# maotian123/loc_lib

Measured on AMD Instinct MI355X. Metric: scans/sec (64x1800-pt scan vs 10M-pt map) + ICP iter ms, higher is better.
Workload: dtype f64; 1 GPU; BASELINE configs[2]: 256 scans/GPU x 115200 pts (64x1800, cityblock-v1) vs one 10000000-pt map, P2PLANE ICP, reference defaults (alpha=0.1 KD-tree ANN, eps=1e-2, max 20 iters), scans sharded by rank, no collective; includes scan H2D: every step aligns a batch copied host->HBM for it (pinned double buffer, copy stream, overlapped with the previous step); 3 alignment(s) in flight; scans_per_gpu=256, map_points=10000000, pipeline_depth=3, search_mode=tree_faithful_ann, tree_depth=30, tree_bytes=239999992

## Files before the change

include/locgpu.h:

```cpp
#ifndef LOCGPU_H_
#define LOCGPU_H_

#include <stddef.h>
#include <stdint.h>

#ifdef __cplusplus
extern "C" {
#endif

#define LOCGPU_API __attribute__((visibility("default")))

typedef struct locgpu_ctx locgpu_ctx;
typedef struct locgpu_batch locgpu_batch;

typedef enum locgpu_status {
    LOCGPU_OK = 0,
    LOCGPU_ERR_INVALID = -1,
    LOCGPU_ERR_NO_DEVICE = -2,
    LOCGPU_ERR_NO_TARGET = -3,
    LOCGPU_ERR_K_TOO_LARGE = -4,
    LOCGPU_ERR_DEPTH = -5,
    LOCGPU_ERR_OOM = -6
} locgpu_status;

// ... 185 lines not shown
LOCGPU_API int locgpu_ndt_align(locgpu_ctx* ctx, const void* src, size_t n, size_t stride_bytes, const double init_pose[7],
                                double out_pose[7], locgpu_align_stats* stats);
LOCGPU_API int locgpu_ndt_hb(locgpu_ctx* ctx, const void* src, size_t n, size_t stride_bytes, const double pose[7], double H[36], double B[6],
                             int64_t* effective_num, int* ok);
LOCGPU_API int locgpu_ndt_hb_batch(locgpu_ctx* ctx, locgpu_batch* b, const double* poses, double* hb);

LOCGPU_API int locgpu_ndt_fitness(locgpu_ctx* ctx, const void* src, size_t n, size_t stride_bytes, const double* poses, int n_poses,
                                  locgpu_fitness* out);
LOCGPU_API int locgpu_ndt_fitness_batch(locgpu_ctx* ctx, locgpu_batch* batch, const double* poses, locgpu_fitness* out);
LOCGPU_API int locgpu_ndt_fitness_resident(locgpu_ctx* ctx, const double pose[7], locgpu_fitness* out);
LOCGPU_API int locgpu_ndt_init_search(locgpu_ctx* ctx, const void* src, size_t n, size_t stride_bytes, const double* candidates, int m,
                                      const locgpu_init_search_opts* sopts, double* out_poses, locgpu_fitness* out_fit,
                                      locgpu_align_stats* stats, int* best);

LOCGPU_API int locgpu_graph_enable(locgpu_ctx* ctx, int on);

LOCGPU_API int locgpu_profile_enable(locgpu_ctx* ctx, int on);
LOCGPU_API int locgpu_profile_read(locgpu_ctx* ctx, double out[6], int reset);
LOCGPU_API int locgpu_visit_count_enable(locgpu_ctx* ctx, int on);
LOCGPU_API int locgpu_visit_count_read(locgpu_ctx* ctx, uint64_t out[4], int reset);

LOCGPU_API int locgpu_search_stats_read(locgpu_ctx* ctx, uint64_t out[4], int reset);
LOCGPU_API int locgpu_debug_batch_nn(locgpu_ctx* ctx, locgpu_batch* batch, int k, int32_t* out);

typedef struct locgpu_cloud locgpu_cloud;
typedef struct locgpu_submap locgpu_submap;
#define LOCGPU_NO_INTENSITY ((size_t)-1)

LOCGPU_API int locgpu_cloud_create(locgpu_ctx* ctx, locgpu_cloud** out);
LOCGPU_API void locgpu_cloud_destroy(locgpu_cloud* c);
LOCGPU_API int locgpu_cloud_upload(locgpu_cloud* c, const void* pts, size_t n, size_t stride_bytes, size_t intensity_offset, int is_dense);
LOCGPU_API int locgpu_cloud_info(const locgpu_cloud* c, size_t* n, int* is_dense);
LOCGPU_API int locgpu_cloud_download(const locgpu_cloud* c, void* out, size_t capacity, size_t stride_bytes, size_t intensity_offset);
LOCGPU_API int locgpu_cloud_copy(const locgpu_cloud* in, locgpu_cloud* out);

LOCGPU_API int locgpu_cloud_remove_nan(const locgpu_cloud* in, locgpu_cloud* out);
LOCGPU_API int locgpu_cloud_voxel_filter(const locgpu_cloud* in, float leaf, locgpu_cloud* out, int* passthrough);
LOCGPU_API int locgpu_cloud_crop_box(const locgpu_cloud* in, const float min_xyz[3], const float max_xyz[3], locgpu_cloud* out);
LOCGPU_API int locgpu_cloud_transform(const locgpu_cloud* in, const double pose[7], locgpu_cloud* out);
LOCGPU_API int locgpu_cloud_append(locgpu_cloud* dst, const locgpu_cloud* src);

LOCGPU_API int locgpu_icp_set_target_cloud(locgpu_ctx* ctx, const locgpu_cloud* target);
LOCGPU_API int locgpu_icp_set_target_cloud_async(locgpu_ctx* ctx, const locgpu_cloud* target);
LOCGPU_API int locgpu_ndt_set_target_cloud(locgpu_ctx* ctx, const locgpu_cloud* target, const locgpu_ndt_opts* opts);
LOCGPU_API int locgpu_icp_align_cloud(locgpu_ctx* ctx, const locgpu_cloud* src, const double init_pose[7], const locgpu_icp_opts* opts,
                                      double out_pose[7], locgpu_align_stats* stats);
// ... 62 lines not shown
```

loc_lib_amd/api.py:

```python
import ctypes
import os
import subprocess

import numpy as np

_HERE = os.path.dirname(os.path.abspath(__file__))
LIB_PATH = os.environ.get("LOCGPU_LIB") or os.path.join(_HERE, "liblocgpu.so")
CSRC = os.path.join(_HERE, "csrc")

P2P, P2LINE, P2PLANE = 0, 1, 2
P2PLANE_MAP = 5
SEARCH_TREE_FAITHFUL, SEARCH_GRID_EXACT = 0, 1
CENTER, NEARBY6 = 0, 1
DIRECT_NDT, INCREMENTAL_NDT = 1, 2

ABI_SYMBOLS = [
    "locgpu_icp_opts_default", "locgpu_ndt_opts_default", "locgpu_create", "locgpu_destroy", "locgpu_last_error",
    "locgpu_device_count", "locgpu_icp_set_target", "locgpu_icp_set_target_async", "locgpu_icp_target_info", "locgpu_knn", "locgpu_icp_hb", "locgpu_icp_align",
    "locgpu_transform_cloud", "locgpu_batch_create", "locgpu_batch_destroy", "locgpu_icp_align_batch", "locgpu_ndt_align_batch",
    "locgpu_icp_hb_batch", "locgpu_gn_update", "locgpu_ndt_set_target", "locgpu_ndt_target_info", "locgpu_ndt_dump",
    "locgpu_ndt_align", "locgpu_profile_enable", "locgpu_profile_read", "locgpu_visit_count_enable", "locgpu_visit_count_read",
    "locgpu_search_stats_read", "locgpu_debug_batch_nn", "locgpu_graph_enable",
    "locgpu_cloud_create", "locgpu_cloud_destroy", "locgpu_cloud_upload", "locgpu_cloud_info", "locgpu_cloud_download", "locgpu_cloud_copy",
    "locgpu_cloud_remove_nan", "locgpu_cloud_voxel_filter", "locgpu_cloud_crop_box", "locgpu_cloud_transform", "locgpu_cloud_append",
    "locgpu_icp_set_target_cloud", "locgpu_icp_set_target_cloud_async", "locgpu_ndt_set_target_cloud", "locgpu_icp_align_cloud", "locgpu_ndt_align_cloud",
    "locgpu_voxel_filter", "locgpu_crop_box", "locgpu_remove_nan",
    "locgpu_submap_create", "locgpu_submap_destroy", "locgpu_submap_add_keyframe", "locgpu_submap_cloud", "locgpu_submap_last_keyframe",
    "locgpu_submap_info", "locgpu_cloud_loam_extract", "locgpu_loam_extract",
    "locgpu_batch_create_empty", "locgpu_batch_upload_async", "locgpu_batch_upload_wait",
    "locgpu_bfnn_set_target", "locgpu_bfnn_knn",
    "locgpu_icp_align_batch_begin", "locgpu_ndt_align_batch_begin", "locgpu_align_batch_end",
    "locgpu_comm_unique_id", "locgpu_comm_init", "locgpu_comm_info", "locgpu_batch_create_sharded", "locgpu_icp_set_target_bcast",
    "locgpu_pool_opts_default", "locgpu_pool_create", "locgpu_pool_destroy", "locgpu_pool_submit", "locgpu_pool_wait", "locgpu_pool_info",
    "locgpu_pool_profile_read", "locgpu_pool_step", "locgpu_pool_done",
    "locgpu_icp_scan_match", "locgpu_ndt_scan_match",
    "locgpu_icp_fitness", "locgpu_icp_fitness_batch", "locgpu_icp_fitness_resident", "locgpu_batch_create_shared",
    "locgpu_init_search_opts_default", "locgpu_icp_init_search", "locgpu_pose_grid",
    "locgpu_ndt_fitness", "locgpu_ndt_fitness_batch", "locgpu_ndt_fitness_resident", "locgpu_ndt_init_search", "locgpu_ndt_hb", "locgpu_ndt_hb_batch",
    "locgpu_icp_build_map_planes", "locgpu_icp_map_planes_info", "locgpu_icp_map_planes_dump",
    "locgpu_loam_opts_default", "locgpu_loam_create", "locgpu_loam_destroy", "locgpu_loam_last_error", "locgpu_loam_set_target",
    "locgpu_loam_hb", "locgpu_loam_scan_match", "locgpu_loam_align_batch",
    "locgpu_loam_set_target_cloud", "locgpu_loam_set_target_cloud_async", "locgpu_loam_scan_match_cloud", "locgpu_loam_fitness_resident",
    "locgpu_loam_submap_create", "locgpu_loam_submap_destroy", "locgpu_loam_submap_add_keyframe", "locgpu_loam_submap_clouds", "locgpu_loam_submap_info",
    "locgpu_loam_create_on", "locgpu_loam_fitness", "locgpu_loam_fitness_cloud", "locgpu_loam_init_search", "locgpu_loam_init_search_cloud",
    "locgpu_batch_preprocess", "locgpu_batch_upload_clouds", "locgpu_batch_download_scan",
# ... 62 lines not shown
        if not os.path.exists(LIB_PATH):
            raise LocGpuError(-2, "liblocgpu.so is not built (run `python -c 'import __graft_entry__ as g; g.build()'`); no CPU fallback exists")
        L = ctypes.CDLL(LIB_PATH)
        vp, sz, i32, dbl, f32 = ctypes.c_void_p, ctypes.c_size_t, ctypes.c_int, ctypes.c_double, ctypes.c_float
        sig = {
            "locgpu_icp_opts_default": (None, [vp]), "locgpu_ndt_opts_default": (None, [vp]),
            "locgpu_create": (i32, [i32, vp]), "locgpu_destroy": (None, [vp]), "locgpu_last_error": (ctypes.c_char_p, [vp]),
            "locgpu_device_count": (i32, []),
            "locgpu_icp_set_target": (i32, [vp, vp, sz, sz]), "locgpu_icp_set_target_async": (i32, [vp, vp, sz, sz]), "locgpu_icp_target_info": (i32, [vp, vp]),
            "locgpu_knn": (i32, [vp, vp, sz, i32, i32, f32, i32, vp, vp]),
            "locgpu_icp_hb": (i32, [vp, vp, sz, sz, vp, vp, vp, vp, vp, vp]),
            "locgpu_icp_align": (i32, [vp, vp, sz, sz, vp, vp, vp, vp]),
            "locgpu_transform_cloud": (i32, [vp, vp, vp, sz, sz, vp, sz]),
            "locgpu_batch_create": (i32, [vp, vp, vp, sz, i32, vp]), "locgpu_batch_destroy": (None, [vp]),
            "locgpu_icp_align_batch": (i32, [vp, vp, vp, vp, vp, vp]), "locgpu_ndt_align_batch": (i32, [vp, vp, vp, vp, vp]),
            "locgpu_icp_align_batch_begin": (i32, [vp, vp, vp, vp]), "locgpu_ndt_align_batch_begin": (i32, [vp, vp, vp]),
            "locgpu_align_batch_end": (i32, [vp, vp, vp, vp]),
            "locgpu_icp_hb_batch": (i32, [vp, vp, vp, vp, vp]),
            "locgpu_gn_update": (i32, [vp, i32, i32, dbl, vp, vp, vp, vp]),
            "locgpu_ndt_set_target": (i32, [vp, vp, sz, sz, vp]), "locgpu_ndt_target_info": (i32, [vp, vp]),
            "locgpu_ndt_dump": (i32, [vp, vp, vp, vp, sz, vp]), "locgpu_ndt_align": (i32, [vp, vp, sz, sz, vp, vp, vp]),
            "locgpu_profile_enable": (i32, [vp, i32]), "locgpu_profile_read": (i32, [vp, vp, i32]),
            "locgpu_visit_count_enable": (i32, [vp, i32]), "locgpu_visit_count_read": (i32, [vp, vp, i32]),
            "locgpu_search_stats_read": (i32, [vp, vp, i32]), "locgpu_debug_batch_nn": (i32, [vp, vp, i32, vp]), "locgpu_graph_enable": (i32, [vp, i32]),
            "locgpu_cloud_create": (i32, [vp, vp]), "locgpu_cloud_destroy": (None, [vp]),
            "locgpu_cloud_upload": (i32, [vp, vp, sz, sz, sz, i32]), "locgpu_cloud_info": (i32, [vp, vp, vp]),
            "locgpu_cloud_download": (i32, [vp, vp, sz, sz, sz]), "locgpu_cloud_copy": (i32, [vp, vp]),
            "locgpu_cloud_remove_nan": (i32, [vp, vp]), "locgpu_cloud_voxel_filter": (i32, [vp, f32, vp, vp]),
            "locgpu_cloud_crop_box": (i32, [vp, vp, vp, vp]), "locgpu_cloud_transform": (i32, [vp, vp, vp]),
            "locgpu_cloud_append": (i32, [vp, vp]),
            "locgpu_icp_set_target_cloud": (i32, [vp, vp]), "locgpu_icp_set_target_cloud_async": (i32, [vp, vp]), "locgpu_ndt_set_target_cloud": (i32, [vp, vp, vp]),
            "locgpu_icp_align_cloud": (i32, [vp, vp, vp, vp, vp, vp]), "locgpu_ndt_align_cloud": (i32, [vp, vp, vp, vp, vp]),
            "locgpu_voxel_filter": (i32, [vp, vp, sz, sz, sz, i32, f32, vp, vp, vp]),
            "locgpu_crop_box": (i32, [vp, vp, sz, sz, sz, i32, vp, vp, vp, vp, vp]),
            "locgpu_remove_nan": (i32, [vp, vp, sz, sz, sz, i32, vp, vp, vp]),
            "locgpu_submap_create": (i32, [vp, i32, f32, vp]), "locgpu_submap_destroy": (None, [vp]),
            "locgpu_submap_add_keyframe": (i32, [vp, vp, vp]), "locgpu_submap_cloud": (i32, [vp, vp]),
            "locgpu_submap_last_keyframe": (i32, [vp, vp]), "locgpu_submap_info": (i32, [vp, vp, vp]),
            "locgpu_cloud_loam_extract": (i32, [vp, vp, i32, vp, vp]),
            "locgpu_loam_extract": (i32, [vp, vp, sz, sz, sz, i32, sz, i32, vp, vp, vp, vp, sz, sz]),
            "locgpu_batch_create_empty": (i32, [vp, i32, sz, vp]), "locgpu_batch_upload_async": (i32, [vp, vp, vp, sz]),
            "locgpu_batch_upload_wait": (i32, [vp]),
            "locgpu_comm_unique_id": (i32, [vp]), "locgpu_comm_init": (i32, [vp, i32, i32, vp]), "locgpu_comm_info": (i32, [vp, vp, vp]),
            "locgpu_batch_create_sharded": (i32, [vp, vp, vp, sz, i32, i32, i32, vp]),
            "locgpu_icp_set_target_bcast": (i32, [vp, vp, sz, sz, i32]),
            "locgpu_bfnn_set_target": (i32, [vp, vp, sz, sz]), "locgpu_bfnn_knn": (i32, [vp, vp, sz, i32, vp]),
            "locgpu_pool_opts_default": (None, [vp]), "locgpu_pool_create": (i32, [vp, vp, vp]), "locgpu_pool_destroy": (None, [vp]),
# ... 703 lines not shown

    @staticmethod
    def _marshal(scans):
        if isinstance(scans, MarshalledScans):
            return scans.scans, scans.ptrs, scans.cnts, scans.stride
        scans = [_cloud(s) for s in scans]
        if not scans:
            raise ValueError("empty batch")
        stride = next((s.strides[0] for s in scans if s.shape[0]), 16)
        if any(s.shape[0] and s.strides[0] != stride for s in scans):
            raise ValueError("all scans of a batch must share one point stride")
        ptrs = (ctypes.c_void_p * len(scans))(*[s.ctypes.data for s in scans])
        cnts = (ctypes.c_size_t * len(scans))(*[s.shape[0] for s in scans])
        return scans, ptrs, cnts, stride

    def upload_async(self, scans):
        self.upload_wait()
        scans, ptrs, cnts, stride = self._marshal(scans)
        if len(scans) != self.n_local:
            raise ValueError("upload_async needs %d scans" % self.n_local)
        self._keep = (scans, ptrs, cnts)
        self.ctx._check(lib().locgpu_batch_upload_async(self._h, ptrs, cnts, stride))

    def upload_wait(self):
        if self._keep is not None:
            rc = lib().locgpu_batch_upload_wait(self._h)
            self._keep = None
            self.ctx._check(rc)

    def preprocess(self, leaf, out=None):
        self.upload_wait()
        dst = self if out is None else out
        dst.upload_wait()
        counts, status = np.zeros(self.n_local, np.int32), np.zeros(self.n_local, np.int32)
        rc = lib().locgpu_batch_preprocess(self._h, float(leaf), dst._h, counts.ctypes.data, status.ctypes.data)
        if rc != 0:
            err = LocGpuError(rc, lib().locgpu_last_error(self.ctx._h).decode())
            err.counts = counts
            raise err
        return counts, status

    def loam_extract(self, rings, num_scan, edge, surf):
        self.upload_wait()
        edge.upload_wait()
        surf.upload_wait()
        rings = [np.ascontiguousarray(r, dtype=np.uint8) if r is not None else None for r in rings]
# ... 283 lines not shown
```

loc_lib_amd/csrc/context.hpp:

```cpp
#pragma once
#include <hip/hip_runtime.h>

#include <string>
#include <vector>

#include "../../include/locgpu.h"
#include "batch_upload.hpp"
#include "device_buffer.hpp"
#include "device_math.hpp"
#include "grid_kernels.hpp"
#include "icp_kernels.hpp"

#include "host_worker.hpp"

struct NdtTable;
namespace locgpu {
struct IncNdtState;
struct FilterScratch;
struct LoamScratch;
struct BatchFilterScratch;
struct BatchLoamScratch;
struct MergeScratch;
}

// ... 5 lines not shown
    bool grid = false;
    bool ndt() const { return method_is_ndt(prm.method); }
    int k() const { return method_k(prm.method); }
    bool operator==(const AlignSpec& o) const { return prm == o.prm && alpha == o.alpha && grid == o.grid; }
};
constexpr int kNdtOptDirect = 1, kNdtOptIncremental = 2;
constexpr int kNearbyCenter = 0, kNearby6 = 1;
constexpr int ndt_n_nearby(int nearby_type) { return nearby_type == kNearbyCenter ? 1 : 7; }
struct StageEvents {
    std::vector<Event> ev;
    size_t used = 0;
    int mode = 0;
    void mark(hipStream_t s, bool search_edge = false);
    void collect(locgpu_ctx* ctx, bool ndt);
};
}

struct locgpu_ctx {
    int device = 0;
    hipStream_t stream = nullptr;
    static constexpr int kSlots = 3;
    hipStream_t slot_stream[kSlots] = {};
    int next_slot = 0;
    hipStream_t copy_stream = nullptr;
    locgpu::Event foreign_ev;
    hipStream_t comm_stream = nullptr;
    locgpu::Uploader* up = nullptr;
    locgpu::PendingTarget* target_scratch = nullptr;
    locgpu::PendingTarget* pending_target = nullptr;
    std::string err;

    locgpu::DevBuf<uint2> d_tree;
    size_t tree_slots = 0, num_leaves = 0, num_nodes = 0, num_points = 0;
    int depth = 0;
    bool tree_bounded = true;
    unsigned long long target_epoch = 0;

    locgpu::DevBuf<uint32_t> d_leaf_slots;

    locgpu::DevBuf<double> d_planes;
    size_t planes_rows = 0;
    bool planes_ready = false;
    long long planes_valid = 0;
    locgpu::DevBuf<unsigned long long> d_planes_count;
    locgpu_batch* planes_ws = nullptr;

// ... 16 lines not shown
    locgpu_batch* single = nullptr;
    size_t single_cap = 0;
    locgpu_batch* search = nullptr;
    locgpu::HostWorker* worker = nullptr;

    void* comm = nullptr;
    int comm_rank = 0, comm_world = 1;

    int profile = 0;
    double prof_ms[3] = {0, 0, 0};
    long long prof_n[3] = {0, 0, 0};
    bool use_graph = false;
    bool count_visits = false;
    locgpu::DevBuf<unsigned long long> d_visits;
    locgpu::DevBuf<uint32_t> d_touched;
    size_t touched_words = 0;
    locgpu::DevBuf<unsigned long long> d_search_stats;
};

struct locgpu_batch {
    locgpu_ctx* ctx = nullptr;
    int slot = 0;
    hipStream_t stream = nullptr;
    int n_scans = 0, max_n = 0, blocks_per_scan = 0;
    int n_total = 0, first = 0;
    bool sharded = false;
    locgpu::DevBuf<double> d_acc;
    size_t pitch = 0;
    locgpu::DevBuf<float4> d_src;
    locgpu::DevBuf<int> d_counts;
    locgpu::DevBuf<locgpu::PoseState> d_state;
    locgpu::DevBuf<uint32_t> d_nn;
    bool shared_src = false;
    locgpu::DevBuf<int> d_src_of;
    int cap_scans = 0, split_scans = 0;
    size_t cap_points = 0;
    const float4* d_src_ext = nullptr;
    bool counters_clean = false;
    int last_iterations = -1;
    locgpu::DevBuf<double> d_partials;
    locgpu::DevBuf<double> d_hb;
    locgpu::DevBuf<uint32_t> d_redo_list;
    locgpu::DevBuf<unsigned int> d_redo_count;
    locgpu::DevBuf<uint32_t> d_redo_list2;
    locgpu::DevBuf<uint32_t> d_grid_qkey;
    locgpu::DevBuf<uint2> d_grid_sorted;
// ... 59 lines not shown
```

loc_lib_amd/csrc/gn_driver.hip:

```cpp
#include <algorithm>
#include <chrono>
#include <cmath>
#include <cstdlib>
#include <cstring>
#include <string>
#include <thread>

#include "batch_upload.hpp"
#include "env.hpp"
#include "gn_driver.hpp"
#include "ndt_inc.hpp"
#include "ndt_kernels.hpp"

namespace locgpu {

namespace {
inline int next_chunk(const locgpu_batch* b) { return b->n_total == 1 ? 2 : kNextChunk; }
inline int first_chunk_len(const locgpu_batch* b) {
    if (b->n_total != 1 || b->sharded || b->last_iterations < 0) return kFirstChunk;
    return std::min(kLongFirstChunk, std::max(3, b->last_iterations + 1));
}

}

SearchArgs make_search_args(const locgpu_ctx* ctx, const locgpu_batch* b, const float4* src, const PoseState* st, int k, float alpha_eff, bool skip_nonfinite) {
    SearchArgs sa{ctx->d_tree, ctx->tree_slots * sizeof(uint64_t), ctx->depth, src, b->d_counts, st, b->d_nn, b->pitch, b->max_n, b->n_scans, k, alpha_eff,
                  skip_nonfinite ? 1 : 0, nullptr, b->d_redo_list, b->d_redo_count, b->d_redo_list2, b->d_redo_count + 1, ctx->d_search_stats};
    if (!ctx->tree_bounded) sa.redo_list = nullptr;
    return sa;
}

void init_state(PoseState& ps, const double pose[7]) {
    std::memset(&ps, 0, sizeof(ps));
    for (int i = 0; i < 4; ++i) ps.q[i] = pose[i];
    for (int i = 0; i < 3; ++i) ps.t[i] = pose[4 + i];
// ... 189 lines not shown
}

static int ensure_graphs(locgpu_ctx* ctx, locgpu_batch* b, const AlignSpec& spec) {
    const void* target = !spec.ndt() ? (const void*)ctx->d_tree : (spec.prm.method == kMethodNdtInc ? inc_ndt_table_ptr(ctx->inc) : (const void*)ctx->ndt->d_rec);
    if (b->graph_exec && b->graph_spec == spec && b->graph_target == target && b->graph_epoch == ctx->target_epoch) return LOCGPU_OK;
    const int first = std::min(kFirstChunk, spec.prm.max_iteration);
    if (b->graph_exec) { (void)hipGraphExecDestroy(b->graph_exec); b->graph_exec = nullptr; }
    if (b->graph_exec_next) { (void)hipGraphExecDestroy(b->graph_exec_next); b->graph_exec_next = nullptr; }
    int rc = capture_chunk(ctx, b, spec, first, true, &b->graph_exec);
    if (rc == LOCGPU_OK && spec.prm.max_iteration > first) rc = capture_chunk(ctx, b, spec, next_chunk(b), false, &b->graph_exec_next);
    if (rc != LOCGPU_OK) return rc;
    b->graph_spec = spec; b->graph_target = target;
    b->graph_epoch = ctx->target_epoch;
    return LOCGPU_OK;
}

static int enqueue_chunk(locgpu_ctx* ctx, locgpu_batch* b, bool first_chunk) {
    locgpu_batch::Pending& P = b->pending;
    const GnParams& prm = P.spec.prm;
    hipStream_t s = b->stream;
    if (P.graph) {
        LOCGPU_HIP(ctx, hipGraphLaunch(first_chunk ? b->graph_exec : b->graph_exec_next, s));
        P.launched += first_chunk ? std::min(kFirstChunk, prm.max_iteration) : next_chunk(b);
        return LOCGPU_OK;
    }
    if (first_chunk) LOCGPU_HIP(ctx, hipMemcpyAsync(b->d_state, b->h_state, b->n_total * sizeof(PoseState), hipMemcpyHostToDevice, s));
    IterLauncher it{ctx, b, P.spec};
    if (!first_chunk && !P.spec.ndt() && b->n_scans > 1) {
        int na = 0;
        for (int i = 0; i < b->n_scans; ++i)
            if (!b->h_state[b->first + i].done) b->h_active[na++] = i;
        if (na > 0 && na < b->n_scans) {
            LOCGPU_HIP(ctx, hipMemcpyAsync(b->d_active, b->h_active, (size_t)na * sizeof(int), hipMemcpyHostToDevice, s));
            it.active = b->d_active;
            it.n_active = na;
        }
    }
    const int todo = std::min(first_chunk ? first_chunk_len(b) : next_chunk(b), prm.max_iteration - P.launched);
    for (int c = 0; c < todo; ++c)
        if (!it.launch(1)) return LOCGPU_ERR_NO_DEVICE;
    P.launched += todo;
    if (it.replicated_on_comm_stream) {
        LOCGPU_HIP(ctx, hipEventRecord(b->ev_reduced, ctx->comm_stream));
        LOCGPU_HIP(ctx, hipStreamWaitEvent(s, b->ev_reduced, 0));
    }
    LOCGPU_HIP(ctx, hipMemcpyAsync(b->h_state, b->d_state, b->n_total * sizeof(PoseState), hipMemcpyDeviceToHost, s));
    return LOCGPU_OK;
}

inline int pace_ahead() {
    static const int v = std::max(0, std::min(8, env_int("LOCGPU_PACE_AHEAD", 1)));
    return v;
}

static int paced_launch(locgpu_ctx* ctx, locgpu_batch* b, int upto) {
    locgpu_batch::Pending& P = b->pending;
    IterLauncher it{ctx, b, P.spec};
    const GnPost post{reinterpret_cast<GnPostRecord*>(b->h_post.get()), b->h_post + locgpu_batch::kPostWord, b->post_call};
    it.post = &post;
    while (P.launched < upto) {
        if (!it.launch(1)) return LOCGPU_ERR_NO_DEVICE;
        P.launched++;
    }
    return LOCGPU_OK;
}

constexpr int kPacedTimeoutS = 30;
static int paced_wait(locgpu_ctx* ctx, locgpu_batch* b, int seen, unsigned long long* out) {
    auto fresh = [&](unsigned long long* w_out) {
// ... 16 lines not shown
        return true;
    };
    const auto t0 = std::chrono::steady_clock::now();
    for (unsigned long spins = 1;; ++spins) {
        if (fresh(out)) return LOCGPU_OK;
#if defined(__x86_64__)
        __builtin_ia32_pause();
#endif
        if ((spins & 0xffff) == 0 && std::chrono::steady_clock::now() - t0 > std::chrono::milliseconds(200)) {
            const hipError_t q = hipStreamQuery(b->stream);
            if (q == hipErrorNotReady) {
                if (std::chrono::steady_clock::now() - t0 > std::chrono::seconds(kPacedTimeoutS))
                    return fail(ctx, LOCGPU_ERR_NO_DEVICE, "paced alignment: no post from the solve kernel within the time-out (the stream is still busy)");
                std::this_thread::yield();
                continue;
            }
            if (q != hipSuccess) { hip_ok(ctx, q, "paced alignment"); return LOCGPU_ERR_NO_DEVICE; }
            if (fresh(out)) return LOCGPU_OK;
            return fail(ctx, LOCGPU_ERR_NO_DEVICE, "paced alignment: the stream is idle and the solve kernel's post has not arrived");
        }
    }
}

int align_begin(locgpu_ctx* ctx, locgpu_batch* b, const double* init_poses, const AlignSpec& spec, bool blocking) {
    const GnParams& prm = spec.prm;
    const bool ndt = spec.ndt();
    LOCGPU_HIP(ctx, hipSetDevice(ctx->device));
    locgpu_batch::Pending& P = b->pending;
    if (P.active) return fail(ctx, LOCGPU_ERR_INVALID, "align: an alignment of this batch has been begun and not finished");
    if (!ndt) { const int grc = ensure_grid_lists(ctx, b, spec); if (grc != LOCGPU_OK) return grc; }
    { const int urc = batch_ready(ctx, b); if (urc != LOCGPU_OK) return urc; }
    P.spec = spec;
    P.graph = ctx->use_graph && !ctx->count_visits && !b->sharded && prm.max_iteration > 0;
    P.launched = 0;
    b->stage_ev.used = 0;
    P.init_poses.assign(init_poses, init_poses + 7 * (size_t)b->n_total);
    init_states(b, init_poses);
    if (!ndt && !b->counters_clean) LOCGPU_HIP(ctx, hipMemsetAsync(b->d_redo_count, 0, 4 * sizeof(unsigned int), b->stream));
    b->counters_clean = false;
    if (P.graph) { const int rc = ensure_graphs(ctx, b, spec); if (rc != LOCGPU_OK) return rc; }
    P.paced = blocking && !P.graph && b->n_total == 1 && !b->sharded && !ctx->profile && !ctx->count_visits && prm.max_iteration > 0 && pace_ahead() > 0 && !spec.grid;
    if (P.paced) {
        if (!b->h_post) {
            LOCGPU_HIP(ctx, b->h_post.alloc(256 / sizeof(unsigned long long), hipHostMallocCoherent));
            std::memset(b->h_post, 0, 256);
        }
        b->post_call++;
        LOCGPU_HIP(ctx, hipMemcpyAsync(b->d_state, b->h_state, sizeof(PoseState), hipMemcpyHostToDevice, b->stream));
        const int rc = paced_launch(ctx, b, std::min(prm.max_iteration, 1 + pace_ahead()));
        if (rc != LOCGPU_OK) { (void)hipStreamSynchronize(b->stream); return rc; }
    } else if (prm.max_iteration > 0) {
        const int rc = enqueue_chunk(ctx, b, true);
        if (rc != LOCGPU_OK) return rc;
    }
    P.active = true;
    return LOCGPU_OK;
}

int align_finish(locgpu_ctx* ctx, locgpu_batch* b, double* out_poses, locgpu_align_stats* stats) {
    LOCGPU_HIP(ctx, hipSetDevice(ctx->device));
    locgpu_batch::Pending& P = b->pending;
    if (!P.active) return fail(ctx, LOCGPU_ERR_INVALID, "align: no alignment of this batch has been begun");
    const int max_iteration = P.spec.prm.max_iteration;
    P.active = false;
    if (P.paced) {
        int seen = 0;
        for (;;) {
            unsigned long long w = 0;
            int rc = paced_wait(ctx, b, seen, &w);
            if (rc == LOCGPU_OK) {
                seen = (int)((w & 0xffffffffull) >> 1);
                if ((w & 1ull) || seen >= max_iteration) break;
                rc = paced_launch(ctx, b, std::min(max_iteration, seen + 1 + pace_ahead()));
            }
            if (rc != LOCGPU_OK) { (void)hipStreamSynchronize(b->stream); return rc; }
        }
        b->paced_tail = true;
    }
    while (!P.paced && max_iteration > 0) {
        LOCGPU_HIP(ctx, hipStreamSynchronize(b->stream));
        b->stage_ev.collect(ctx, P.spec.ndt());
        bool all_done = true;
        for (int i = 0; i < b->n_total; ++i)
            if (!b->h_state[i].done) { all_done = false; break; }
        if (all_done || P.launched >= max_iteration) break;
        const int rc = enqueue_chunk(ctx, b, false);
        if (rc != LOCGPU_OK) {
            (void)hipStreamSynchronize(b->stream);
            return rc;
        }
    }
    for (int i = 0; i < b->n_total; ++i) write_scan_result(b->h_state[i], P.init_poses.data() + 7 * (size_t)i, out_poses + 7 * (size_t)i, stats ? stats + i : nullptr);
    b->counters_clean = !P.spec.ndt() && !ctx->count_visits && !P.spec.grid && !b->sharded;
    if (b->n_total == 1 && max_iteration > 0) b->last_iterations = b->h_state[0].iterations;
    return LOCGPU_OK;
}

int run_align(locgpu_ctx* ctx, locgpu_batch* b, const double* init_poses, const AlignSpec& spec, double* out_poses, locgpu_align_stats* stats) {
    const int rc = align_begin(ctx, b, init_poses, spec,  true);
    return rc != LOCGPU_OK ? rc : align_finish(ctx, b, out_poses, stats);
}

constexpr size_t kPlaneChunk = (size_t)1 << 20;
int ensure_map_planes(locgpu_ctx* ctx) {
    if (ctx->planes_ready) return LOCGPU_OK;
    LOCGPU_HIP(ctx, hipSetDevice(ctx->device));
    hipStream_t s = ctx->stream;
    const size_t rows = ctx->tree_slots / 2 + 2;
    if (rows * 4 > ctx->d_planes.cap() && !hip_ok(ctx, ctx->d_planes.alloc(with_headroom(rows) * 4), "hipMalloc map planes")) return LOCGPU_ERR_OOM;
    if (!hip_ok(ctx, ctx->d_planes_count.reserve(1), "hipMalloc map planes")) return LOCGPU_ERR_OOM;
    LOCGPU_HIP(ctx, hipMemsetAsync(ctx->d_planes, 0xFF, rows * 4 * sizeof(double), s));
    LOCGPU_HIP(ctx, hipMemsetAsync(ctx->d_planes_count, 0, sizeof(unsigned long long), s));
    unsigned long long n_valid = 0;
    if (ctx->num_leaves >= 5) {
        const size_t chunk = std::min(ctx->num_leaves, kPlaneChunk);
        locgpu_batch* w = ctx->planes_ws;
        if (!w || (size_t)w->max_n < chunk) {
            if (w) { free_batch(w); ctx->planes_ws = nullptr; }
            const int next_slot = ctx->next_slot;
            const int rc = alloc_batch(ctx, 1, chunk, &ctx->planes_ws);
            ctx->next_slot = next_slot;
            if (rc != LOCGPU_OK) return rc;
            w = ctx->planes_ws;
            w->slot = 0;
            w->stream = s;
        }
        const double identity[7] = {0, 0, 0, 1, 0, 0, 0};
        init_states(w, identity);
        LOCGPU_HIP(ctx, hipMemsetAsync(w->d_redo_count, 0, 4 * sizeof(unsigned int), s));
        LOCGPU_HIP(ctx, hipMemcpyAsync(w->d_state, w->h_state, sizeof(PoseState), hipMemcpyHostToDevice, s));
        for (size_t first = 0; first < ctx->num_leaves; first += chunk) {
            const int cnt = (int)std::min(chunk, ctx->num_leaves - first);
            launch_map_plane_queries(ctx->d_tree, ctx->d_leaf_slots, first, cnt, w->d_src, w->d_counts, s);
            SearchArgs sa = make_search_args(ctx, w, w->d_src, w->d_state, 5, 1.0f, false);
            sa.search_stats = nullptr;
            if (!launch_icp_search(sa, s)) return fail(ctx, LOCGPU_ERR_DEPTH, "icp_build_map_planes: unsupported tree depth");
            LOCGPU_HIP(ctx, hipMemsetAsync(w->d_redo_count, 0, 4 * sizeof(unsigned int), s));
            launch_map_plane_fit(ctx->d_tree, ctx->d_leaf_slots, first, cnt, w->d_nn, w->pitch, ctx->d_planes, ctx->d_planes_count, s);
        }
        LOCGPU_HIP(ctx, hipGetLastError());
        LOCGPU_HIP(ctx, hipMemcpyAsync(&n_valid, ctx->d_planes_count, sizeof(n_valid), hipMemcpyDeviceToHost, s));
    }
    LOCGPU_HIP(ctx, hipStreamSynchronize(s));
    ctx->planes_rows = ctx->num_leaves;
    ctx->planes_valid = (long long)n_valid;
    ctx->planes_ready = true;
    return LOCGPU_OK;
}
// ... 75 lines not shown
```

loc_lib_amd/csrc/loam_align.hip:

```cpp
#include <algorithm>
#include <cmath>
#include <cstring>
#include <string>
#include <vector>

#include "batch_upload.hpp"
#include "cloud_filters.hpp"
#include "context.hpp"
#include "gn_driver.hpp"
#include "launch.hpp"
#include "search_chunks.hpp"

using namespace locgpu;

namespace {
constexpr int kSurf = 0, kEdge = 1;
}

struct locgpu_loam {
    int device = 0;
    locgpu_loam_opts opts{};
    bool use[2] = {false, false};
    locgpu_ctx* ctx[2] = {nullptr, nullptr};
    bool borrowed = false;
// ... 71 lines not shown
                    lhip(l, l->d_active.alloc((size_t)n), "hipMalloc active") &&
                    lhip(l, l->h_active.alloc((size_t)n), "hipHostMalloc active") &&
                    lhip(l, l->d_fit.alloc((size_t)n * 3 * kFitW), "hipMalloc fit") &&
                    lhip(l, l->h_fit.alloc((size_t)n * 3 * kFitW), "hipHostMalloc fit");
    return ok ? LOCGPU_OK : LOCGPU_ERR_OOM;
}

int shape_batch(locgpu_loam* l, int c, int n_scans, size_t max_n) {
    locgpu_ctx* ctx = l->ctx[c];
    locgpu_batch* b = l->batch[c];
    max_n = std::max<size_t>(max_n, 1);
    if (!b || b->cap_scans < n_scans || b->cap_points < max_n) {
        const int cs = std::max(n_scans, b ? b->cap_scans : 0);
        size_t cp = std::max(max_n, b ? b->cap_points : (size_t)0);
        if (cp == max_n && n_scans == 1) cp = with_headroom(max_n);
        if (b) { (void)hipStreamSynchronize(l->stream); free_batch(b); l->batch[c] = nullptr; }
        const int slot = ctx->next_slot;
        int rc = from_ctx(l, c, alloc_batch(ctx, cs, cp, &l->batch[c]));
        ctx->next_slot = slot;
        if (rc != LOCGPU_OK) return rc;
        b = l->batch[c];
        b->slot = 0;
        b->stream = ctx->stream;
        if (!lhip(l, b->upl.h_counts.alloc((size_t)cs), "hipHostMalloc counts")) return LOCGPU_ERR_OOM;
    }
    if (b->n_scans != n_scans || (size_t)b->max_n != max_n) {
        if ((size_t)n_scans * max_n > b->pitch) {
            b->d_grid_qkey.reset();
            b->d_grid_sorted.reset();
        }
        b->n_scans = b->n_total = n_scans;
        b->max_n = (int)max_n;
        b->blocks_per_scan = (int)((max_n + kBlock - 1) / kBlock);
        b->pitch = (size_t)n_scans * max_n;
        b->counts.assign(n_scans, 0);
    }
    return LOCGPU_OK;
}

int upload_scans(locgpu_loam* l, int n_scans, const void* const* srcs[2], const size_t* counts[2], size_t stride) {
    size_t max_n[2] = {0, 0};
    l->src_of[kSurf] = l->src_of[kEdge] = nullptr;
    l->split_scans = 0;
    for (int c = 0; c < 2; ++c) {
        if (!l->use[c]) continue;
        if (!srcs[c] || !counts[c]) return lfail(l, LOCGPU_ERR_INVALID, "loam: the scans of an enabled feature class are NULL");
// ... 729 lines not shown
```

loc_lib_amd/csrc/locgpu_api.hip:

```cpp
#include <algorithm>
#include <atomic>
#include <cmath>
#include <cstdio>
#include <cstdlib>
#include <cstring>
#include <string>
#include <vector>

#include "batch_upload.hpp"
#include "cloud_filters.hpp"
#include "context.hpp"
#include "gn_driver.hpp"
#include "launch.hpp"
#include "ndt_inc.hpp"
#include "ndt_kernels.hpp"
#include "search_chunks.hpp"

using namespace locgpu;

namespace {
std::string g_create_err;
}

namespace locgpu {
int fail(locgpu_ctx* ctx, int code, const std::string& msg) {
    if (ctx) ctx->err = msg;
    else g_create_err = msg;
    return code;
}
bool hip_ok(locgpu_ctx* ctx, hipError_t e, const char* what) {
    if (e == hipSuccess) return true;
    fail(ctx, LOCGPU_ERR_NO_DEVICE, std::string(what) + ": " + hipGetErrorString(e));
    return false;
}
}

static bool fill_now(locgpu_ctx* ctx, void* p, size_t bytes, const char* what) {
    return hip_ok(ctx, hipMemsetAsync(p, 0, bytes, ctx->stream), what) && hip_ok(ctx, hipStreamSynchronize(ctx->stream), what);
}

void locgpu::free_batch(locgpu_batch* b) {
    if (!b) return;
    upload_free_batch(b);
    if (b->graph_exec) (void)hipGraphExecDestroy(b->graph_exec);
    if (b->graph_exec_next) (void)hipGraphExecDestroy(b->graph_exec_next);
    delete b;
}

extern "C" {

void locgpu_icp_opts_default(locgpu_icp_opts* o) {
    if (!o) return;
    o->method = LOCGPU_P2P;
    o->max_iteration = 20;
    o->max_nn_distance = 1.0;
    o->max_plane_distance = 0.1;
    o->max_line_distance = 0.5;
    o->min_effective_pts = 10;
    o->eps = 1e-2;
    o->approximate = 1;
    o->ann_alpha = 0.1f;
    o->search_mode = LOCGPU_SEARCH_TREE_FAITHFUL;
}

void locgpu_ndt_opts_default(locgpu_ndt_opts* o) {
    if (!o) return;
// ... 281 lines not shown
    prm.max_nn_distance = o->max_nn_distance;
    prm.max_plane_distance = o->max_plane_distance;
    prm.max_line_distance = o->max_line_distance;
    if (o->method == LOCGPU_P2PLANE_MAP) {
        const int rc = ensure_map_planes(ctx);
        if (rc != LOCGPU_OK) return rc;
    }
    spec.grid = o->search_mode == LOCGPU_SEARCH_GRID_EXACT;
    spec.alpha = (o->approximate && !spec.grid) ? o->ann_alpha : 1.0f;
    return LOCGPU_OK;
}

static int single_reserve(locgpu_ctx* ctx, size_t n, locgpu_batch** out) {
    if (n == 0) return fail(ctx, LOCGPU_ERR_INVALID, "source cloud is empty");
    locgpu_batch* b = ctx->single;
    if (!b || (size_t)b->max_n < n || !b->h_src) {
        if (b) { free_batch(b); ctx->single = nullptr; }
        const size_t cap = with_headroom(n);
        const int rc = alloc_batch(ctx, 1, cap, &ctx->single);
        if (rc != LOCGPU_OK) return rc;
        b = ctx->single;
        b->slot = 0;
        b->stream = ctx->stream;
        if (!hip_ok(ctx, b->h_src.alloc(cap), "hipHostMalloc src")) { free_batch(b); ctx->single = nullptr; return LOCGPU_ERR_OOM; }
    }
    *out = b;
    return LOCGPU_OK;
}

static int single_batch(locgpu_ctx* ctx, const void* src, size_t n, size_t stride_bytes, locgpu_batch** out) {
    if (n == 0) return fail(ctx, LOCGPU_ERR_INVALID, "source cloud is empty");
    if (!src || stride_bytes < 12) return fail(ctx, LOCGPU_ERR_INVALID, "source cloud: NULL pointer or stride < 12");
    locgpu_batch* b = nullptr;
    const int rc = single_reserve(ctx, n, &b);
    if (rc != LOCGPU_OK) return rc;
    pack_points((const char*)src, stride_bytes, n, b->h_src);
    b->d_src_ext = nullptr;
    b->counts[0] = (int)n;
    LOCGPU_HIP(ctx, hipMemcpyAsync(b->d_src, b->h_src, n * sizeof(float4), hipMemcpyHostToDevice, b->stream));
    LOCGPU_HIP(ctx, hipMemcpyAsync(b->d_counts, b->counts.data(), sizeof(int), hipMemcpyHostToDevice, b->stream));
    *out = b;
    return LOCGPU_OK;
}

static int single_batch_dev(locgpu_ctx* ctx, const float4* d_src, size_t n, locgpu_batch** out) {
    locgpu_batch* b = nullptr;
// ... 297 lines not shown

int upload_shared(locgpu_ctx* ctx, locgpu_batch* b, const void* src, size_t n, size_t stride_bytes) {
    if (!b->h_src) LOCGPU_HIP(ctx, b->h_src.alloc(b->cap_points));
    pack_points((const char*)src, stride_bytes, n, b->h_src);
    LOCGPU_HIP(ctx, hipMemcpyAsync(b->d_src, b->h_src, n * sizeof(float4), hipMemcpyHostToDevice, b->stream));
    return LOCGPU_OK;
}

int search_batch(locgpu_ctx* ctx, const void* src, size_t n, size_t stride_bytes, int m, int* chunk, locgpu_batch** out) {
    *chunk = search_chunk(kSearchBytesPerPoint * n, m);
    locgpu_batch* b = ctx->search;
    if (!b || b->cap_scans < *chunk || b->cap_points < n) {
        int cs = std::max(*chunk, b ? b->cap_scans : 0);
        size_t cp = std::max(n, b ? b->cap_points : (size_t)0);
        if ((size_t)cs * cp * kSearchBytesPerPoint > kSearchBytes) { cs = *chunk; cp = n; }
        if (b) { (void)hipStreamSynchronize(b->stream); free_batch(b); ctx->search = nullptr; }
        const int slot = ctx->next_slot;
        const int rc = alloc_batch(ctx, cs, cp, &ctx->search, 0, -1, true);
        ctx->next_slot = slot;
        if (rc != LOCGPU_OK) return rc;
        b = ctx->search;
        b->slot = 0;
        b->stream = ctx->stream;
    }
    const int rc = upload_shared(ctx, b, src, n, stride_bytes);
    if (rc != LOCGPU_OK) return rc;
    *out = b;
    return LOCGPU_OK;
}

int fitness_target(locgpu_ctx* ctx) {
    { const int jrc = target_join(ctx); if (jrc != LOCGPU_OK) return jrc; }
    if (!ctx->d_tree) return fail(ctx, LOCGPU_ERR_NO_TARGET, "icp_fitness: SetInputTarget has not been called");
    return LOCGPU_OK;
}

int ndt_fitness_target(locgpu_ctx* ctx, const char* who) {
    if (ctx->ndt_opts.method == kNdtOptIncremental) {
        if (!ctx->inc) return fail(ctx, LOCGPU_ERR_NO_TARGET, std::string(who) + ": SetInputTarget has not been called");
        return fail(ctx, LOCGPU_ERR_INVALID, std::string(who) + ": the current NDT target is the incremental one (method 2); the score and the search are defined for the direct target only");
    }
    if (!ctx->ndt) return fail(ctx, LOCGPU_ERR_NO_TARGET, std::string(who) + ": SetInputTarget has not been called");
    return LOCGPU_OK;
}

template <class Score>
// ... 163 lines not shown
        return true;
    };
    long kxy = 0, kyaw = 0;
    if (!steps(xy_half, xy_step, &kxy) || !steps(yaw_half, yaw_step, &kyaw)) return LOCGPU_ERR_INVALID;
    const size_t nxy = (size_t)(2 * kxy + 1), nyaw = (size_t)(2 * kyaw + 1);
    *n_out = nyaw * nxy * nxy;
    double R[9];
    quat_to_R(centre, R);
    size_t w = 0;
    for (long a = -kyaw; a <= kyaw && w < cap; ++a) {
        const double yaw = (double)a * yaw_step, sz = std::sin(0.5 * yaw), cz = std::cos(0.5 * yaw);
        const double q[4] = {centre[0] * cz + centre[1] * sz, centre[1] * cz - centre[0] * sz, centre[2] * cz + centre[3] * sz, centre[3] * cz - centre[2] * sz};
        for (long ix = -kxy; ix <= kxy && w < cap; ++ix)
            for (long iy = -kxy; iy <= kxy && w < cap; ++iy) {
                const double x = (double)ix * xy_step, y = (double)iy * xy_step;
                double* o = out + 7 * w++;
                for (int j = 0; j < 4; ++j) o[j] = q[j];
                for (int r = 0; r < 3; ++r) o[4 + r] = centre[4 + r] + (R[3 * r] * x + R[3 * r + 1] * y);
            }
    }
    return LOCGPU_OK;
}

int locgpu_graph_enable(locgpu_ctx* ctx, int on) {
    if (!ctx) return LOCGPU_ERR_INVALID;
    ctx->use_graph = on != 0;
    return LOCGPU_OK;
}

int locgpu_profile_enable(locgpu_ctx* ctx, int on) {
    if (!ctx) return LOCGPU_ERR_INVALID;
    ctx->profile = on == 2 ? 2 : (on != 0 ? 1 : 0);
    return LOCGPU_OK;
}

int locgpu_profile_read(locgpu_ctx* ctx, double out[6], int reset) {
    if (!ctx || !out) return LOCGPU_ERR_INVALID;
    for (int j = 0; j < 3; ++j) {
        out[j] = ctx->prof_n[j] ? ctx->prof_ms[j] / (double)ctx->prof_n[j] : 0.0;
        out[3 + j] = (double)ctx->prof_n[j];
    }
    if (reset)
        for (int j = 0; j < 3; ++j) { ctx->prof_ms[j] = 0; ctx->prof_n[j] = 0; }
    return LOCGPU_OK;
}

// ... 244 lines not shown
```

Measured before the change: 12250 scans/s.

## Lease slot streams dynamically to batches at align begin by least load

Adds a stream-lease scheme: at align_begin a non-pinned batch moves to the least-loaded of the three slot streams, keeping its current one if that is idle, and releases it at finish. When a stream is shared, finish waits on a per-chunk event instead of synchronizing the whole stream. The intent is to stop in-flight alignments from serializing on one stream when batch-to-slot assignment is uneven. It adds event records per chunk and cross-stream waits when a batch migrates.

```diff
diff --git a/include/locgpu.h b/include/locgpu.h
--- a/include/locgpu.h
+++ b/include/locgpu.h
@@ -231,6 +231,7 @@
 
 LOCGPU_API int locgpu_search_stats_read(locgpu_ctx* ctx, uint64_t out[4], int reset);
 LOCGPU_API int locgpu_debug_batch_nn(locgpu_ctx* ctx, locgpu_batch* batch, int k, int32_t* out);
+LOCGPU_API int locgpu_debug_batch_slot(const locgpu_batch* batch);
 
 typedef struct locgpu_cloud locgpu_cloud;
 typedef struct locgpu_submap locgpu_submap;
diff --git a/loc_lib_amd/api.py b/loc_lib_amd/api.py
--- a/loc_lib_amd/api.py
+++ b/loc_lib_amd/api.py
@@ -20,7 +20,7 @@
     "locgpu_transform_cloud", "locgpu_batch_create", "locgpu_batch_destroy", "locgpu_icp_align_batch", "locgpu_ndt_align_batch",
     "locgpu_icp_hb_batch", "locgpu_gn_update", "locgpu_ndt_set_target", "locgpu_ndt_target_info", "locgpu_ndt_dump",
     "locgpu_ndt_align", "locgpu_profile_enable", "locgpu_profile_read", "locgpu_visit_count_enable", "locgpu_visit_count_read",
-    "locgpu_search_stats_read", "locgpu_debug_batch_nn", "locgpu_graph_enable",
+    "locgpu_search_stats_read", "locgpu_debug_batch_nn", "locgpu_debug_batch_slot", "locgpu_graph_enable",
     "locgpu_cloud_create", "locgpu_cloud_destroy", "locgpu_cloud_upload", "locgpu_cloud_info", "locgpu_cloud_download", "locgpu_cloud_copy",
     "locgpu_cloud_remove_nan", "locgpu_cloud_voxel_filter", "locgpu_cloud_crop_box", "locgpu_cloud_transform", "locgpu_cloud_append",
     "locgpu_icp_set_target_cloud", "locgpu_icp_set_target_cloud_async", "locgpu_ndt_set_target_cloud", "locgpu_icp_align_cloud", "locgpu_ndt_align_cloud",
@@ -129,7 +129,7 @@
             "locgpu_ndt_dump": (i32, [vp, vp, vp, vp, sz, vp]), "locgpu_ndt_align": (i32, [vp, vp, sz, sz, vp, vp, vp]),
             "locgpu_profile_enable": (i32, [vp, i32]), "locgpu_profile_read": (i32, [vp, vp, i32]),
             "locgpu_visit_count_enable": (i32, [vp, i32]), "locgpu_visit_count_read": (i32, [vp, vp, i32]),
-            "locgpu_search_stats_read": (i32, [vp, vp, i32]), "locgpu_debug_batch_nn": (i32, [vp, vp, i32, vp]), "locgpu_graph_enable": (i32, [vp, i32]),
+            "locgpu_search_stats_read": (i32, [vp, vp, i32]), "locgpu_debug_batch_nn": (i32, [vp, vp, i32, vp]), "locgpu_debug_batch_slot": (i32, [vp]), "locgpu_graph_enable": (i32, [vp, i32]),
             "locgpu_cloud_create": (i32, [vp, vp]), "locgpu_cloud_destroy": (None, [vp]),
             "locgpu_cloud_upload": (i32, [vp, vp, sz, sz, sz, i32]), "locgpu_cloud_info": (i32, [vp, vp, vp]),
             "locgpu_cloud_download": (i32, [vp, vp, sz, sz, sz]), "locgpu_cloud_copy": (i32, [vp, vp]),
@@ -879,6 +879,9 @@
         self._keep = (scans, ptrs, cnts)
         self.ctx._check(lib().locgpu_batch_upload_async(self._h, ptrs, cnts, stride))
 
+    def debug_slot(self):
+        return int(lib().locgpu_debug_batch_slot(self._h))
+
     def upload_wait(self):
         if self._keep is not None:
             rc = lib().locgpu_batch_upload_wait(self._h)
diff --git a/loc_lib_amd/csrc/context.hpp b/loc_lib_amd/csrc/context.hpp
--- a/loc_lib_amd/csrc/context.hpp
+++ b/loc_lib_amd/csrc/context.hpp
@@ -51,6 +51,7 @@
     static constexpr int kSlots = 3;
     hipStream_t slot_stream[kSlots] = {};
     int next_slot = 0;
+    int slot_load[kSlots] = {};
     hipStream_t copy_stream = nullptr;
     locgpu::Event foreign_ev;
     hipStream_t comm_stream = nullptr;
@@ -113,6 +114,9 @@
     locgpu_ctx* ctx = nullptr;
     int slot = 0;
     hipStream_t stream = nullptr;
+    bool pinned = false;
+    bool leased = false;
+    locgpu::Event chunk_ev;
     int n_scans = 0, max_n = 0, blocks_per_scan = 0;
     int n_total = 0, first = 0;
     bool sharded = false;
diff --git a/loc_lib_amd/csrc/gn_driver.hip b/loc_lib_amd/csrc/gn_driver.hip
--- a/loc_lib_amd/csrc/gn_driver.hip
+++ b/loc_lib_amd/csrc/gn_driver.hip
@@ -11,6 +11,7 @@
 #include "gn_driver.hpp"
 #include "ndt_inc.hpp"
 #include "ndt_kernels.hpp"
+#include "stream_lease.hpp"
 
 namespace locgpu {
 
@@ -246,6 +247,7 @@
     if (P.graph) {
         LOCGPU_HIP(ctx, hipGraphLaunch(first_chunk ? b->graph_exec : b->graph_exec_next, s));
         P.launched += first_chunk ? std::min(kFirstChunk, prm.max_iteration) : next_chunk(b);
+        LOCGPU_HIP(ctx, hipEventRecord(b->chunk_ev, s));
         return LOCGPU_OK;
     }
     if (first_chunk) LOCGPU_HIP(ctx, hipMemcpyAsync(b->d_state, b->h_state, b->n_total * sizeof(PoseState), hipMemcpyHostToDevice, s));
@@ -269,6 +271,7 @@
         LOCGPU_HIP(ctx, hipStreamWaitEvent(s, b->ev_reduced, 0));
     }
     LOCGPU_HIP(ctx, hipMemcpyAsync(b->h_state, b->d_state, b->n_total * sizeof(PoseState), hipMemcpyDeviceToHost, s));
+    LOCGPU_HIP(ctx, hipEventRecord(b->chunk_ev, s));
     return LOCGPU_OK;
 }
 
@@ -331,12 +334,34 @@
     }
 }
 
-int align_begin(locgpu_ctx* ctx, locgpu_batch* b, const double* init_poses, const AlignSpec& spec, bool blocking) {
+static int lease_take(locgpu_ctx* ctx, locgpu_batch* b) {
+    if (b->pinned) return LOCGPU_OK;
+    const int to = lease_choose(ctx->slot_load, locgpu_ctx::kSlots, b->slot);
+    if (to != b->slot) {
+        if (b->paced_tail) {
+            LOCGPU_HIP(ctx, b->tail_ev.ensure());
+            LOCGPU_HIP(ctx, hipEventRecord(b->tail_ev, b->stream));
+            LOCGPU_HIP(ctx, hipStreamWaitEvent(ctx->slot_stream[to], b->tail_ev, 0));
+        }
+        b->slot = to;
+        b->stream = ctx->slot_stream[to];
+    }
+    ctx->slot_load[to]++;
+    b->leased = true;
+    return LOCGPU_OK;
+}
+
+static void lease_release(locgpu_ctx* ctx, locgpu_batch* b) {
+    if (!b->leased) return;
+    ctx->slot_load[b->slot]--;
+    b->leased = false;
+}
+
+static int begin_on_stream(locgpu_ctx* ctx, locgpu_batch* b, const double* init_poses, const AlignSpec& spec, bool blocking) {
     const GnParams& prm = spec.prm;
     const bool ndt = spec.ndt();
-    LOCGPU_HIP(ctx, hipSetDevice(ctx->device));
     locgpu_batch::Pending& P = b->pending;
-    if (P.active) return fail(ctx, LOCGPU_ERR_INVALID, "align: an alignment of this batch has been begun and not finished");
+    LOCGPU_HIP(ctx, b->chunk_ev.ensure());
     if (!ndt) { const int grc = ensure_grid_lists(ctx, b, spec); if (grc != LOCGPU_OK) return grc; }
     { const int urc = batch_ready(ctx, b); if (urc != LOCGPU_OK) return urc; }
     P.spec = spec;
@@ -366,12 +391,21 @@
     return LOCGPU_OK;
 }
 
-int align_finish(locgpu_ctx* ctx, locgpu_batch* b, double* out_poses, locgpu_align_stats* stats) {
+int align_begin(locgpu_ctx* ctx, locgpu_batch* b, const double* init_poses, const AlignSpec& spec, bool blocking) {
     LOCGPU_HIP(ctx, hipSetDevice(ctx->device));
+    if (b->pending.active) return fail(ctx, LOCGPU_ERR_INVALID, "align: an alignment of this batch has been begun and not finished");
+    { const int lrc = lease_take(ctx, b); if (lrc != LOCGPU_OK) return lrc; }
+    const int rc = begin_on_stream(ctx, b, init_poses, spec, blocking);
+    if (rc != LOCGPU_OK) {
+        (void)hipStreamSynchronize(b->stream);
+        lease_release(ctx, b);
+    }
+    return rc;
+}
+
+static int finish_on_stream(locgpu_ctx* ctx, locgpu_batch* b, double* out_poses, locgpu_align_stats* stats) {
     locgpu_batch::Pending& P = b->pending;
-    if (!P.active) return fail(ctx, LOCGPU_ERR_INVALID, "align: no alignment of this batch has been begun");
     const int max_iteration = P.spec.prm.max_iteration;
-    P.active = false;
     if (P.paced) {
         int seen = 0;
         for (;;) {
@@ -387,7 +421,12 @@
         b->paced_tail = true;
     }
     while (!P.paced && max_iteration > 0) {
-        LOCGPU_HIP(ctx, hipStreamSynchronize(b->stream));
+        const bool shared = ctx->slot_load[b->slot] > (b->leased ? 1 : 0);
+        if (const hipError_t e = shared ? hipEventSynchronize(b->chunk_ev) : hipStreamSynchronize(b->stream); e != hipSuccess) {
+            (void)hipStreamSynchronize(b->stream);
+            hip_ok(ctx, e, "align: waiting for the chunk");
+            return LOCGPU_ERR_NO_DEVICE;
+        }
         b->stage_ev.collect(ctx, P.spec.ndt());
         bool all_done = true;
         for (int i = 0; i < b->n_total; ++i)
@@ -403,6 +442,15 @@
     b->counters_clean = !P.spec.ndt() && !ctx->count_visits && !P.spec.grid && !b->sharded;
     if (b->n_total == 1 && max_iteration > 0) b->last_iterations = b->h_state[0].iterations;
     return LOCGPU_OK;
+}
+
+int align_finish(locgpu_ctx* ctx, locgpu_batch* b, double* out_poses, locgpu_align_stats* stats) {
+    LOCGPU_HIP(ctx, hipSetDevice(ctx->device));
+    if (!b->pending.active) return fail(ctx, LOCGPU_ERR_INVALID, "align: no alignment of this batch has been begun");
+    b->pending.active = false;
+    const int rc = finish_on_stream(ctx, b, out_poses, stats);
+    lease_release(ctx, b);
+    return rc;
 }
 
 int run_align(locgpu_ctx* ctx, locgpu_batch* b, const double* init_poses, const AlignSpec& spec, double* out_poses, locgpu_align_stats* stats) {
@@ -433,6 +481,7 @@
             w = ctx->planes_ws;
             w->slot = 0;
             w->stream = s;
+            w->pinned = true;
         }
         const double identity[7] = {0, 0, 0, 1, 0, 0, 0};
         init_states(w, identity);
diff --git a/loc_lib_amd/csrc/loam_align.hip b/loc_lib_amd/csrc/loam_align.hip
--- a/loc_lib_amd/csrc/loam_align.hip
+++ b/loc_lib_amd/csrc/loam_align.hip
@@ -117,6 +117,7 @@
         b = l->batch[c];
         b->slot = 0;
         b->stream = ctx->stream;
+        b->pinned = true;
         if (!lhip(l, b->upl.h_counts.alloc((size_t)cs), "hipHostMalloc counts")) return LOCGPU_ERR_OOM;
     }
     if (b->n_scans != n_scans || (size_t)b->max_n != max_n) {
diff --git a/loc_lib_amd/csrc/locgpu_api.hip b/loc_lib_amd/csrc/locgpu_api.hip
--- a/loc_lib_amd/csrc/locgpu_api.hip
+++ b/loc_lib_amd/csrc/locgpu_api.hip
@@ -42,6 +42,7 @@
 void locgpu::free_batch(locgpu_batch* b) {
     if (!b) return;
     upload_free_batch(b);
+    if (b->leased) b->ctx->slot_load[b->slot]--;
     if (b->graph_exec) (void)hipGraphExecDestroy(b->graph_exec);
     if (b->graph_exec_next) (void)hipGraphExecDestroy(b->graph_exec_next);
     delete b;
@@ -369,6 +370,7 @@
         b = ctx->single;
         b->slot = 0;
         b->stream = ctx->stream;
+        b->pinned = true;
         if (!hip_ok(ctx, b->h_src.alloc(cap), "hipHostMalloc src")) { free_batch(b); ctx->single = nullptr; return LOCGPU_ERR_OOM; }
     }
     *out = b;
@@ -712,6 +714,7 @@
         b = ctx->search;
         b->slot = 0;
         b->stream = ctx->stream;
+        b->pinned = true;
     }
     const int rc = upload_shared(ctx, b, src, n, stride_bytes);
     if (rc != LOCGPU_OK) return rc;
@@ -921,6 +924,8 @@
     return LOCGPU_OK;
 }
 
+int locgpu_debug_batch_slot(const locgpu_batch* b) { return b ? b->slot : -1; }
+
 int locgpu_graph_enable(locgpu_ctx* ctx, int on) {
     if (!ctx) return LOCGPU_ERR_INVALID;
     ctx->use_graph = on != 0;
diff --git a/loc_lib_amd/csrc/stream_lease.hpp b/loc_lib_amd/csrc/stream_lease.hpp
--- /dev/null
+++ b/loc_lib_amd/csrc/stream_lease.hpp
@@ -0,0 +1,13 @@
+#pragma once
+
+namespace locgpu {
+
+inline int lease_choose(const int* load, int n, int current) {
+    if (current >= 0 && current < n && load[current] == 0) return current;
+    int best = 0;
+    for (int i = 1; i < n; ++i)
+        if (load[i] < load[best]) best = i;
+    return best;
+}
+
+}
```

Result: faster. 12720 scans/s (median of 6 runs) (+3.8%).
